# EavianWoo/SinGS

Measured on AMD Instinct MI355X. Metric: rendered views/sec fwd+bwd, 200k Gaussians @1080p, higher is better.
Workload: dtype f32; 1 GPU; S(200000,1920,1080,deg=3,seed=3): 200000 Gaussians, 1920x1080, SH deg 3, fwd+bwd, R=780064 (tile,Gaussian) pairs, every view of a step within 0.1 % of that (cameras a few cm apart), frame-parallel dp1; gaussians=200000, width=1920, height=1080, sh_degree=3, num_rendered=780064, tile_list_max=135, frames_per_launch=8, streams=2, regularisers=False, forward_only=False, hip_graph=False, reduction=fold of 2 gradient row(s) for 16 views + collective in 1 chunk(s), gradient_rows=2, parallelism=dp1

## Files before the change

### sings_amd/csrc/sg_render_fwd.inc

```

#define SG_TW_BATCH 64
#define SG_TWSORT_MAX 512
static_assert(SG_TWSORT_MAX * 8 == SG_TW_BATCH * 64 && SG_RANKSORT_MAX * 2 * 8 <= SG_TW_BATCH * 64, "sort buffers alias the wave's rows");
static_assert(SG_FB % SG_TW_BATCH == 0, "boxes and checkpoints are refreshed between batches");

#define SG_FWD_TW_QUAD(Q)                                                                                  \
    do {                                                                                                   \
        const float dx = ga.x - (((Q) & 1) ? pxf1 : pxf0), dy = ga.y - (((Q) >> 1) ? pyf1 : pyf0);         \
        const float power = sg_power2(ga.z, ga.w, gb.x, dx, dy);                                           \
        const float alpha = fminf(0.99f, gb.y * __builtin_amdgcn_exp2f(power));                            \
        const float test_T = Tr4[Q] * (1.0f - alpha);                                                      \
        const unsigned long long valid = __ballot(!(power > 0.0f)) & __ballot(!(alpha < 1.0f / 255.0f)) & ~dn4[Q]; \
        const unsigned long long term = valid & __ballot(test_T < 0.0001f);                                \
        const bool blend = __builtin_amdgcn_inverse_ballot_w64(valid & ~term);                             \
        const float w = blend ? alpha * Tr4[Q] : 0.0f;                                                     \
        C04[Q] = fmaf(gb.z, w, C04[Q]); C14[Q] = fmaf(gb.w, w, C14[Q]); C24[Q] = fmaf(gm.x, w, C24[Q]);    \
        if (AUX) Dz4[Q] = fmaf(gm.y, w, Dz4[Q]);                                                           \
        Tr4[Q] = blend ? test_T : Tr4[Q];                                                                  \
        last4[Q] = blend ? pos1 : last4[Q];                                                                \
        dn4[Q] |= term;                                                                                    \
    } while (0)

__device__ __forceinline__ float sg_uniform(float x) { return __uint_as_float(__builtin_amdgcn_readfirstlane(__float_as_uint(x))); }

__device__ __forceinline__ uint32_t sg_list_id(const uint32_t *p) { return __hip_atomic_load(p, __ATOMIC_RELAXED, __HIP_MEMORY_SCOPE_AGENT); }

template <bool AUX>
__device__ __forceinline__ void sg_render_fwd_tile_wave(SG_FWD_PARAMS, SgAuxFwd ax = SgAuxFwd{})
{
    __shared__ float4 sR[4][SG_TW_BATCH][4];
    (void)nblocks; (void)long_items; (void)mask_plane; (void)plan; (void)item_w; (void)w_plane;
    const int tid = threadIdx.x, lane = tid & 63;
    const int wave = __builtin_amdgcn_readfirstlane(tid >> 6);
    if (tid == 0 && blockIdx.x == 0) header[2] = 0u;
    const int tile0 = 4 * sg_tile_of_block((int)blockIdx.x);
    if (tile0 >= T) return;
    const bool overflow = header[1] != 0u;
    {
        bool coop = false;
#pragma unroll
        for (int w = 0; w < 4; w++) {
            const uint2 r = ranges[tile0 + w < T ? tile0 + w : T - 1];
            const int nw = overflow ? 0 : (int)(r.y - r.x);
            coop |= nw > SG_TWSORT_MAX && nw <= SG_WSORT_MAX;
        }
        if (coop) {
            static_assert((SG_WSORT_MAX + SG_RANKSORT_MAX) * 8 <= 4 * SG_TW_BATCH * 64, "the workgroup's sort buffers alias the four waves' rows");
            uint64_t *sKey = (uint64_t *)sR;
            for (int w = 0; w < 4; w++) {
                if (tile0 + w >= T) break;
                const uint2 r = ranges[tile0 + w];
                const int nw = (int)(r.y - r.x);
                if (!(nw > SG_TWSORT_MAX && nw <= SG_WSORT_MAX)) continue;
                sg_sort_short_list(key_pitch ? pair_keys + (size_t)(tile0 + w) * key_pitch : pair_keys + r.x, nw, sKey, sKey + SG_WSORT_MAX, tid);
                for (int i = tid; i < nw; i += 256) {
                    const uint64_t key = sKey[i];
                    point_list[r.x + i] = (uint32_t)key;
                    if (point_keys) point_keys[r.x + i] = ((uint64_t)(tile0 + w) << 32) | (key >> 32);
                }
                __syncthreads();
            }
            __threadfence_block();
        }
    }
    const int tile = tile0 + wave;
    if (tile >= T) return;
    if (lane == 0) tile_count[sg_ctr_of_tile((uint32_t)tile, (uint32_t)gx)] = 0u;
    const int X0 = (tile % gx) * 16, Y0 = (tile / gx) * 16;
    const uint2 range = ranges[tile];
    const int n = overflow ? 0 : (int)(range.y - range.x);
    const uint32_t cks = n > SG_SEG ? ck_start[tile] : 0xffffffffu;
    const int px0 = X0 + (lane & 7), py0 = Y0 + (lane >> 3);
    const float pxf0 = (float)px0, pyf0 = (float)py0, pxf1 = pxf0 + 8.0f, pyf1 = pyf0 + 8.0f;
    float Tr4[4], C04[4], C14[4], C24[4], Dz4[4];
    uint32_t last4[4];
    unsigned long long dn4[4];
#pragma unroll
    for (int q = 0; q < 4; q++) {
        Tr4[q] = 1.0f; C04[q] = 0.0f; C14[q] = 0.0f; C24[q] = 0.0f; Dz4[q] = 0.0f; last4[q] = 0u;
        dn4[q] = __ballot(!(px0 + 8 * (q & 1) < W && py0 + 8 * (q >> 1) < H));
    }
    float4 (*row)[4] = sR[wave];
    float4 pa = make_float4(0, 0, 0, 0), pb = pa;
    float pc = 0.0f, pz = 0.0f;
    if (n > 0 && n <= SG_TWSORT_MAX) {
        uint64_t *sKey = (uint64_t *)row;
        sg_sort_short_list_wave(key_pitch ? pair_keys + (size_t)tile * key_pitch : pair_keys + range.x, n, sKey, lane);
        for (int i = lane; i < n; i += SG_TW_BATCH) {
            const uint64_t key = sKey[i];
            const uint32_t gid = (uint32_t)key;
            point_list[range.x + i] = gid;
            if (point_keys) point_keys[range.x + i] = ((uint64_t)tile << 32) | (key >> 32);
            if (i == lane) {
                pa = recA[SG_REC_STRIDE * (size_t)gid]; pb = recB[SG_REC_STRIDE * (size_t)gid]; pc = recC[SG_REC_STRIDE * (size_t)gid].x;
                if (AUX) pz = ax.depth[gid];
            }
        }
        if (n > SG_TW_BATCH) __threadfence_block();
    } else if (lane < n) {
        const uint32_t gid = sg_list_id(point_list + range.x + lane);
        pa = recA[SG_REC_STRIDE * (size_t)gid]; pb = recB[SG_REC_STRIDE * (size_t)gid]; pc = recC[SG_REC_STRIDE * (size_t)gid].x;
        if (AUX) pz = ax.depth[gid];
    }
    float4 box[4];
    const float X0f = sg_uniform((float)X0), Y0f = sg_uniform((float)Y0);
    for (int base = 0; base < n; base += SG_TW_BATCH) {
        if ((base & (SG_FB - 1)) == 0) {
#pragma unroll
            for (int q = 0; q < 4; q++) {
                const float4 b = sg_live_box(~dn4[q], q);
                box[q] = make_float4(sg_uniform(b.x), sg_uniform(b.y), sg_uniform(b.z), sg_uniform(b.w));
            }
            if ((dn4[0] & dn4[1] & dn4[2] & dn4[3]) == ~0ull) break;
            if (base > 0 && cks != 0xffffffffu && cks + (uint32_t)(base / SG_SEG) < ck_cap) {
                int ln = lane;
                asm volatile("" : "+v"(ln));
                const size_t slot = (size_t)(cks + (uint32_t)(base / SG_SEG)) * 256 + (uint32_t)ln;
#pragma unroll
                for (int q = 0; q < 4; q++)
                    if (dn4[q] != ~0ull) {
                        ckpt[slot + q * 64] = make_float4(Tr4[q], C04[q], C14[q], C24[q]);
                        if (AUX) ax.ckD[slot + q * 64] = Dz4[q];
                    }
            }
        }
        const int e = base + lane;
        uint32_t mk = 0u;
        if (e < n) {
            mk = sg_quad_mask(pa, pb, X0f, Y0f, box);
            row[lane][0] = make_float4(pa.x, pa.y, SG_KA * pa.z, SG_KB * pa.w);
            row[lane][1] = make_float4(SG_KA * pb.x, pb.y, pb.z, pb.w);
            row[lane][2] = make_float4(pc, pz, __uint_as_float(mk), 0.0f);
            pair_mask[range.x + e] = (uint8_t)mk;
        }
        if (e + SG_TW_BATCH < n) {
            const uint32_t gid = sg_list_id(point_list + range.x + e + SG_TW_BATCH);
            pa = recA[SG_REC_STRIDE * (size_t)gid]; pb = recB[SG_REC_STRIDE * (size_t)gid]; pc = recC[SG_REC_STRIDE * (size_t)gid].x;
            if (AUX) pz = ax.depth[gid];
        }
        unsigned long long todo = __ballot(mk != 0u);
        __builtin_amdgcn_wave_barrier();
        while (todo) {
            const int k = __builtin_ctzll(todo);
            todo &= todo - 1ull;
            const float4 ga = row[k][0], gb = row[k][1], gm = row[k][2];
            const uint32_t mke = __builtin_amdgcn_readfirstlane(__float_as_uint(gm.z));
            uint32_t pos1;
            asm volatile("v_mov_b32 %0, %1" : "=v"(pos1) : "s"(base + k + 1));
            if (mke & 1u) SG_FWD_TW_QUAD(0);
            if (mke & 2u) SG_FWD_TW_QUAD(1);
            if (mke & 4u) SG_FWD_TW_QUAD(2);
            if (mke & 8u) SG_FWD_TW_QUAD(3);
        }
        __builtin_amdgcn_wave_barrier();
    }
    const size_t hw = (size_t)H * W;
    const float bg0 = bg[0], bg1 = bg[1], bg2 = bg[2];
    int ln = lane;
    asm volatile("" : "+v"(ln));
#pragma unroll
    for (int q = 0; q < 4; q++) {
        if (cks < ck_cap) {
            ckpt[(size_t)cks * 256 + q * 64 + ln] = make_float4(Tr4[q], C04[q], C14[q], C24[q]);
            if (AUX) ax.ckD[(size_t)cks * 256 + q * 64 + ln] = Dz4[q];
        }
        const int px = X0 + (ln & 7) + 8 * (q & 1), py = Y0 + (ln >> 3) + 8 * (q >> 1);
        if (px < W && py < H) {
            const size_t pid = (size_t)py * W + px;
            final_T[pid] = Tr4[q];
            n_contrib[pid] = last4[q];
            out_color[pid] = fmaf(Tr4[q], bg0, C04[q]);
            out_color[hw + pid] = fmaf(Tr4[q], bg1, C14[q]);
            out_color[2 * hw + pid] = fmaf(Tr4[q], bg2, C24[q]);
            if (AUX) { ax.out_depth[pid] = Dz4[q]; ax.out_alpha[pid] = 1.0f - Tr4[q]; }
        }
    }
}

#undef SG_FWD_TW_QUAD
```

### sings_amd/csrc/sg_sort.h

```cpp
#pragma once
#include "sg_common.h"

#define SG_WSORT_MAX 1024
static_assert(SG_WSORT_MAX == SG_TILE_KEY_CAP, "a row of SgBin::tile_keys holds what a compositing workgroup sorts");
#define SG_RANKSORT_MAX 128

__device__ __forceinline__ void sg_bitonic_wave(uint64_t *__restrict__ s, int n2, int lane)
{
    for (int k = 2; k <= n2; k <<= 1)
        for (int j = k >> 1; j > 0; j >>= 1) {
            for (int t = lane; t < (n2 >> 1); t += 64) {
                const int i = ((t & ~(j - 1)) << 1) | (t & (j - 1)), ixj = i | j;
                const bool up = (i & k) == 0;
                const uint64_t a = s[i], b = s[ixj];
                if ((a > b) == up) { s[i] = b; s[ixj] = a; }
            }
            __builtin_amdgcn_s_waitcnt(0xC07F);
            __builtin_amdgcn_wave_barrier();
        }
}

__device__ __forceinline__ void sg_sort_short_list_wave(const uint64_t *__restrict__ src, int n, uint64_t *__restrict__ s, int lane)
{
    if (n <= SG_RANKSORT_MAX) {
        uint64_t *tmp = s + SG_RANKSORT_MAX;
        uint64_t key0 = 0, key1 = 0;
        if (lane < n) { key0 = src[lane]; tmp[lane] = key0; }
        if (lane + 64 < n) { key1 = src[lane + 64]; tmp[lane + 64] = key1; }
        __builtin_amdgcn_s_waitcnt(0xC07F);
        __builtin_amdgcn_wave_barrier();
        int rank0 = 0, rank1 = 0, j = 0;
        if (n <= 64) {
            for (; j + 2 <= n; j += 2) {
                const ulonglong2 kk = *(const ulonglong2 *)(tmp + j);
                rank0 += (kk.x < key0) + (kk.y < key0);
            }
            if (j < n) rank0 += tmp[j] < key0;
        } else {
            for (; j + 2 <= n; j += 2) {
                const ulonglong2 kk = *(const ulonglong2 *)(tmp + j);
                rank0 += (kk.x < key0) + (kk.y < key0);
                rank1 += (kk.x < key1) + (kk.y < key1);
            }
            if (j < n) { const uint64_t k = tmp[j]; rank0 += k < key0; rank1 += k < key1; }
        }
        if (lane < n) s[rank0] = key0;
        if (lane + 64 < n) s[rank1] = key1;
        __builtin_amdgcn_s_waitcnt(0xC07F);
        __builtin_amdgcn_wave_barrier();
        return;
    }
    int n2 = 1; while (n2 < n) n2 <<= 1;
    for (int i = lane; i < n2; i += 64) s[i] = i < n ? src[i] : ~0ull;
    __builtin_amdgcn_s_waitcnt(0xC07F);
    __builtin_amdgcn_wave_barrier();
    sg_bitonic_wave(s, n2, lane);
}

__device__ __forceinline__ void sg_sort_short_list(const uint64_t *__restrict__ src, int n, uint64_t *__restrict__ s,
                                                   uint64_t *__restrict__ tmp, int tid)
{
    if (n <= SG_RANKSORT_MAX) {
        uint64_t key = 0;
        if (tid < n) { key = src[tid]; tmp[tid] = key; }
        __syncthreads();
        if (tid < n) {
            int rank = 0;
            int j = 0;
            for (; j + 2 <= n; j += 2) {
                const ulonglong2 kk = *(const ulonglong2 *)(tmp + j);
                rank += (kk.x < key) + (kk.y < key);
            }
            if (j < n) rank += tmp[j] < key;
            s[rank] = key;
        }
        __syncthreads();
        return;
    }
    int n2 = 1; while (n2 < n) n2 <<= 1;
    for (int i = tid; i < n2; i += 256) s[i] = i < n ? src[i] : ~0ull;
    __syncthreads();
    if (n2 <= 256) {
        if (tid < 64) sg_bitonic_wave(s, n2, tid);
        __syncthreads();
        return;
    }
    for (int k = 2; k <= n2; k <<= 1)
        for (int j = k >> 1; j > 0; j >>= 1) {
            for (int t = tid; t < (n2 >> 1); t += 256) {
                const int i = ((t & ~(j - 1)) << 1) | (t & (j - 1)), ixj = i | j;
                const bool up = (i & k) == 0;
                const uint64_t a = s[i], b = s[ixj];
                if ((a > b) == up) { s[i] = b; s[ixj] = a; }
            }
            __syncthreads();
        }
}
```

Measured before the change: 5366 views/s.

## Rank-sort short tile lists on 32-bit depth keys with fallback, prefetch second batch ids

The per-wave rank sort for short tile lists now counts ranks using only the upper 32 bits (depth) of each key, with hand-written compare/add-carry assembly over 16 keys per iteration, instead of full 64-bit comparisons. A ballot check catches scatter collisions from equal depths and falls back to the original 64-bit rank pass. The forward kernel also keeps the Gaussian id for the second batch from the sort loop, so the first prefetch does not reread point_list, and the block fence now applies only for lists longer than two batches. This trades a cheaper common path for extra LDS space and an occasional second pass on depth ties.

```diff
diff --git a/sings_amd/csrc/sg_render_fwd.inc b/sings_amd/csrc/sg_render_fwd.inc
--- a/sings_amd/csrc/sg_render_fwd.inc
+++ b/sings_amd/csrc/sg_render_fwd.inc
@@ -1,7 +1,7 @@
 
 #define SG_TW_BATCH 64
 #define SG_TWSORT_MAX 512
-static_assert(SG_TWSORT_MAX * 8 == SG_TW_BATCH * 64 && SG_RANKSORT_MAX * 2 * 8 <= SG_TW_BATCH * 64, "sort buffers alias the wave's rows");
+static_assert(SG_TWSORT_MAX * 8 == SG_TW_BATCH * 64 && SG_RANKSORT_LDS <= SG_TW_BATCH * 64, "sort buffers alias the wave's rows");
 static_assert(SG_FB % SG_TW_BATCH == 0, "boxes and checkpoints are refreshed between batches");
 
 #define SG_FWD_TW_QUAD(Q)                                                                                  \
@@ -83,6 +83,7 @@
     float4 (*row)[4] = sR[wave];
     float4 pa = make_float4(0, 0, 0, 0), pb = pa;
     float pc = 0.0f, pz = 0.0f;
+    uint32_t gid1 = 0u;
     if (n > 0 && n <= SG_TWSORT_MAX) {
         uint64_t *sKey = (uint64_t *)row;
         sg_sort_short_list_wave(key_pitch ? pair_keys + (size_t)tile * key_pitch : pair_keys + range.x, n, sKey, lane);
@@ -94,13 +95,14 @@
             if (i == lane) {
                 pa = recA[SG_REC_STRIDE * (size_t)gid]; pb = recB[SG_REC_STRIDE * (size_t)gid]; pc = recC[SG_REC_STRIDE * (size_t)gid].x;
                 if (AUX) pz = ax.depth[gid];
-            }
+            } else if (i == lane + SG_TW_BATCH) gid1 = gid;
         }
-        if (n > SG_TW_BATCH) __threadfence_block();
+        if (n > 2 * SG_TW_BATCH) __threadfence_block();
     } else if (lane < n) {
         const uint32_t gid = sg_list_id(point_list + range.x + lane);
         pa = recA[SG_REC_STRIDE * (size_t)gid]; pb = recB[SG_REC_STRIDE * (size_t)gid]; pc = recC[SG_REC_STRIDE * (size_t)gid].x;
         if (AUX) pz = ax.depth[gid];
+        if (lane + SG_TW_BATCH < n) gid1 = sg_list_id(point_list + range.x + lane + SG_TW_BATCH);
     }
     float4 box[4];
     const float X0f = sg_uniform((float)X0), Y0f = sg_uniform((float)Y0);
@@ -134,7 +136,8 @@
             pair_mask[range.x + e] = (uint8_t)mk;
         }
         if (e + SG_TW_BATCH < n) {
-            const uint32_t gid = sg_list_id(point_list + range.x + e + SG_TW_BATCH);
+            const uint32_t gid = base == 0 ? gid1 : sg_list_id(point_list + range.x + e + SG_TW_BATCH);
+            gid1 = 0u;
             pa = recA[SG_REC_STRIDE * (size_t)gid]; pb = recB[SG_REC_STRIDE * (size_t)gid]; pc = recC[SG_REC_STRIDE * (size_t)gid].x;
             if (AUX) pz = ax.depth[gid];
         }
diff --git a/sings_amd/csrc/sg_sort.h b/sings_amd/csrc/sg_sort.h
--- a/sings_amd/csrc/sg_sort.h
+++ b/sings_amd/csrc/sg_sort.h
@@ -20,30 +20,64 @@
         }
 }
 
+#define SG_COUNT_BELOW4(R, W, D)                                                                               \
+    do {                                                                                                       \
+        unsigned long long m0_, m1_, m2_, m3_;                                                                 \
+        asm volatile("v_cmp_lt_u32_e64 %1, %5, %9\n\tv_cmp_lt_u32_e64 %2, %6, %9\n\t"                          \
+                     "v_cmp_lt_u32_e64 %3, %7, %9\n\tv_cmp_lt_u32_e64 %4, %8, %9\n\t"                          \
+                     "v_addc_co_u32_e64 %0, %1, 0, %0, %1\n\tv_addc_co_u32_e64 %0, %2, 0, %0, %2\n\t"          \
+                     "v_addc_co_u32_e64 %0, %3, 0, %0, %3\n\tv_addc_co_u32_e64 %0, %4, 0, %0, %4"              \
+                     : "+v"(R), "=&s"(m0_), "=&s"(m1_), "=&s"(m2_), "=&s"(m3_)                                 \
+                     : "v"((W).x), "v"((W).y), "v"((W).z), "v"((W).w), "v"(D));                                \
+    } while (0)
+
+#define SG_RANKSORT_LDS (SG_RANKSORT_MAX * (2 * 8 + 4))
 __device__ __forceinline__ void sg_sort_short_list_wave(const uint64_t *__restrict__ src, int n, uint64_t *__restrict__ s, int lane)
 {
     if (n <= SG_RANKSORT_MAX) {
         uint64_t *tmp = s + SG_RANKSORT_MAX;
-        uint64_t key0 = 0, key1 = 0;
+        uint32_t *dw = (uint32_t *)(s + 2 * SG_RANKSORT_MAX);
+        uint64_t key0 = ~0ull, key1 = ~0ull;
         if (lane < n) { key0 = src[lane]; tmp[lane] = key0; }
         if (lane + 64 < n) { key1 = src[lane + 64]; tmp[lane + 64] = key1; }
+#ifdef SG_SORT_ABLATE
+        if (lane < n) s[lane] = key0;
+        if (lane + 64 < n) s[lane + 64] = key1;
         __builtin_amdgcn_s_waitcnt(0xC07F);
         __builtin_amdgcn_wave_barrier();
-        int rank0 = 0, rank1 = 0, j = 0;
+        return;
+#endif
+        dw[lane] = (uint32_t)(key0 >> 32); dw[lane + 64] = (uint32_t)(key1 >> 32);
+        __builtin_amdgcn_s_waitcnt(0xC07F);
+        __builtin_amdgcn_wave_barrier();
+        uint32_t rank0 = 0, rank1 = 0;
+        const uint32_t d0 = (uint32_t)(key0 >> 32), d1 = (uint32_t)(key1 >> 32);
         if (n <= 64) {
-            for (; j + 2 <= n; j += 2) {
-                const ulonglong2 kk = *(const ulonglong2 *)(tmp + j);
-                rank0 += (kk.x < key0) + (kk.y < key0);
+            for (int t = 0; t < n; t += 16) {
+                const uint4 w0 = *(const uint4 *)(dw + t), w1 = *(const uint4 *)(dw + t + 4), w2 = *(const uint4 *)(dw + t + 8), w3 = *(const uint4 *)(dw + t + 12);
+                SG_COUNT_BELOW4(rank0, w0, d0); SG_COUNT_BELOW4(rank0, w1, d0); SG_COUNT_BELOW4(rank0, w2, d0); SG_COUNT_BELOW4(rank0, w3, d0);
             }
-            if (j < n) rank0 += tmp[j] < key0;
         } else {
-            for (; j + 2 <= n; j += 2) {
-                const ulonglong2 kk = *(const ulonglong2 *)(tmp + j);
-                rank0 += (kk.x < key0) + (kk.y < key0);
-                rank1 += (kk.x < key1) + (kk.y < key1);
+            for (int t = 0; t < n; t += 16) {
+                const uint4 w0 = *(const uint4 *)(dw + t), w1 = *(const uint4 *)(dw + t + 4), w2 = *(const uint4 *)(dw + t + 8), w3 = *(const uint4 *)(dw + t + 12);
+                SG_COUNT_BELOW4(rank0, w0, d0); SG_COUNT_BELOW4(rank1, w0, d1); SG_COUNT_BELOW4(rank0, w1, d0); SG_COUNT_BELOW4(rank1, w1, d1);
+                SG_COUNT_BELOW4(rank0, w2, d0); SG_COUNT_BELOW4(rank1, w2, d1); SG_COUNT_BELOW4(rank0, w3, d0); SG_COUNT_BELOW4(rank1, w3, d1);
             }
-            if (j < n) { const uint64_t k = tmp[j]; rank0 += k < key0; rank1 += k < key1; }
         }
+        if (lane < n) s[rank0] = key0;
+        if (lane + 64 < n) s[rank1] = key1;
+        __builtin_amdgcn_s_waitcnt(0xC07F);
+        __builtin_amdgcn_wave_barrier();
+        if (__ballot((lane < n && s[rank0] != key0) | (lane + 64 < n && s[rank1] != key1)) == 0ull) return;
+        __builtin_amdgcn_wave_barrier();
+        rank0 = 0; rank1 = 0;
+        int j = 0;
+        for (; j + 2 <= n; j += 2) {
+            const ulonglong2 kk = *(const ulonglong2 *)(tmp + j);
+            rank0 += (kk.x < key0) + (kk.y < key0);
+            rank1 += (kk.x < key1) + (kk.y < key1);
+        }
+        if (j < n) { const uint64_t k = tmp[j]; rank0 += k < key0; rank1 += k < key1; }
         if (lane < n) s[rank0] = key0;
         if (lane + 64 < n) s[rank1] = key1;
         __builtin_amdgcn_s_waitcnt(0xC07F);
```

After: 5394 views/s (median of 3 runs). No clear change (+0.5%).
